# powdr-labs/powdr

Measured on AMD Instinct MI355X. Metric: STARK cells/sec (trace rows x cols) proving guest-keccak [bus interactions (LogUp) inside the proof], higher is better.
Workload: dtype u32 (BabyBear, Montgomery)

## Files before the change

### include/powdr_prover.h

```cpp
#ifndef POWDR_PROVER_H
#define POWDR_PROVER_H

#include <stddef.h>
#include <stdint.h>

#ifdef __cplusplus
extern "C" {
#endif

typedef struct PwProver PwProver;

typedef struct {
    uint32_t num_queries;
    uint32_t pow_bits;
} PwStarkConfig;

PwProver* pw_prover_create(const PwStarkConfig* cfg, uint32_t width, const uint32_t* cons_bytecode,
                           size_t bytecode_len, const uint32_t* cons_spans, size_t n_constraints);
PwProver* pw_prover_create_logup(const PwStarkConfig* cfg, uint32_t width, const uint32_t* cons_bytecode,
                                 size_t bytecode_len, const uint32_t* cons_spans, size_t n_constraints,
                                 const uint32_t* interactions, size_t n_interactions, const uint32_t* inter_spans,
                                 size_t n_inter_spans, const uint32_t* inter_bytecode, size_t inter_bytecode_len);
int pw_prover_trace_root(PwProver* p, const uint32_t* d_trace, uint32_t log_height, uint32_t* root8);
int pw_prover_set_bus_seed(PwProver* p, const uint32_t* seed8);
// ... 225 lines not shown
int pw_prover_stream_log_blocks(const PwProver* p, uint32_t log_height);

int pw_prover_max_constraint_degree(const PwProver* p);

int pw_prover_specialise(PwProver* p);
size_t pw_provers_specialise(PwProver* const* provers, size_t n);
int pw_prover_specialised(const PwProver* p, size_t* n_kernels, size_t* code_bytes, size_t* n_chunks);
size_t pw_jit_generated_source(uint32_t width, const uint32_t* cons_bytecode, size_t bytecode_len, const uint32_t* cons_spans, size_t n_constraints,
                               const uint32_t* interactions, size_t n_interactions, const uint32_t* inter_spans, size_t n_inter_spans,
                               const uint32_t* inter_bytecode, size_t inter_bytecode_len, int which, uint32_t chunk_cost, uint32_t chunks_per_unit,
                               size_t unit, char* buf, size_t cap, char* kernel_name, size_t name_cap, uint32_t* first_chunk, uint32_t* n_chunks,
                               uint32_t* total_chunks);
void pw_jit_cache_stats(uint64_t* units_compiled, uint64_t* units_from_disk);
int pw_jit_compile_check(uint32_t width, const uint32_t* cons_bytecode, size_t bytecode_len, const uint32_t* cons_spans, size_t n_constraints,
                         const uint32_t* interactions, size_t n_interactions, const uint32_t* inter_spans, size_t n_inter_spans,
                         const uint32_t* inter_bytecode, size_t inter_bytecode_len, size_t* n_kernels, size_t* code_bytes, size_t* n_chunks,
                         char* err, size_t err_cap);

uint32_t pw_prover_width(const PwProver* p);

size_t pw_prover_device_bytes(const PwProver* p);


int pw_lde_batch(const uint32_t* d_trace, uint32_t width, uint32_t log_height, uint32_t* d_coeffs, uint32_t* d_lde);

int pw_lde_fused(const uint32_t* d_trace, uint32_t width, uint32_t log_height, uint32_t* d_tmp, uint32_t* d_lde);

int pw_lde_subcoset(const uint32_t* d_coeffs, uint32_t width, uint32_t log_height, uint32_t log_blocks, uint32_t r, uint32_t* d_scale,
                    uint32_t* d_out);

int pw_merkle_commit(const uint32_t* d_matrix, size_t height, uint32_t width, uint32_t* d_digests);

void pw_poseidon2_permute_host(uint32_t* state16);

int pw_set_poseidon2_constants(const uint32_t* ext_rc, const uint32_t* int_rc);
void pw_get_poseidon2_constants(uint32_t* ext_rc, uint32_t* int_rc, uint32_t* diag);

#ifdef __cplusplus
}
#endif
#endif
```

### powdr_amd/csrc/field_selftest.hpp

```cpp
#pragma once
#include "ext.hpp"
#include "poseidon2.hpp"

namespace pw {

PW_HD void selftest_permute_ref(uint32_t* s, const p2::Params& P) {
    auto linear = [&]() {
        uint32_t t[16];
        for (int b = 0; b < 4; ++b) {
            const uint32_t x0 = s[4 * b], x1 = s[4 * b + 1], x2 = s[4 * b + 2], x3 = s[4 * b + 3];
            const uint32_t all = bb::add(bb::add(x0, x1), bb::add(x2, x3));
            t[4 * b] = bb::add(bb::add(all, x0), bb::double_(x1));
            t[4 * b + 1] = bb::add(bb::add(all, x1), bb::double_(x2));
            t[4 * b + 2] = bb::add(bb::add(all, x2), bb::double_(x3));
            t[4 * b + 3] = bb::add(bb::add(all, x3), bb::double_(x0));
        }
        for (int i = 0; i < 4; ++i) {
            const uint32_t col = bb::add(bb::add(t[i], t[4 + i]), bb::add(t[8 + i], t[12 + i]));
            for (int b = 0; b < 4; ++b) s[4 * b + i] = bb::add(t[4 * b + i], col);
        }
    };
    auto sbox = [](uint32_t x) { const uint32_t x2 = bb::mul(x, x), x3 = bb::mul(x2, x), x4 = bb::mul(x2, x2); return bb::mul(x3, x4); };
    linear();
#pragma unroll 1
// ... 168 lines not shown
        }
    }
    if (!params) return 40;
    {
        const uint32_t top = (uint32_t)B::kInputTop - 1;
        const uint32_t mixed[8] = {0u, P - 1, (P - 1) / 2, (P + 1) / 2, P, P + 1, top, 1u};
        const uint32_t n_cases = 2 * (10 + iterations / 64);
#pragma unroll 1
        for (uint32_t c = 0; c < n_cases; ++c) {
            const uint32_t init = c >> 1;
            const int k = (c & 1) ? 3 : 8;
            uint32_t st[16], ref[16], one[16];
            for (int i = 0; i < 16; ++i) {
                st[i] = init == 0 ? 0u : init == 1 ? P - 1 : init == 2 ? (P - 1) / 2 : init == 3 ? (P + 1) / 2 : init == 4 ? mixed[i & 3]
                      : init == 5 ? P : init == 6 ? P + 1 : init == 7 ? top : init == 8 ? mixed[(i * 5 + 4) & 7]
                      : (init & 1) ? rp() : (uint32_t)(rnd() % (uint64_t)B::kInputTop);
                ref[i] = st[i] % P;
            }
#pragma unroll 1
            for (int step = 0; step < 3; ++step) {
                if (step)
                    for (int i = 0; i < k; ++i) st[i] = ref[i] = init < 9 ? mixed[(i + step + init) & 3] : rp();
                for (int i = 0; i < 16; ++i) one[i] = st[i];
                p2::permute<false>(one, *params);
                p2::permute<true>(st, *params);
                selftest_permute_ref(ref, *params);
                for (int i = 0; i < 16; ++i) {
                    if (one[i] != ref[i]) return 38;
                    if (st[i] >= (uint32_t)B::kInputTop || st[i] % P != ref[i]) return 39;
                }
            }
            for (int i = 0; i < 16; ++i)
                if (reduce_2p(st[i]) != ref[i]) return 39;
        }
    }
    for (uint32_t it = 0; it < iterations; ++it) {
        const uint32_t a = rp(), b = rp(), c = rp(), d = rp();
        {
            const int32_t x = (int32_t)((int64_t)(rnd() % (2ull * P + P / 11)) - (int64_t)(P + P / 22));
            uint32_t want = R_MOD_P;
            for (int k = 0; k < 7; ++k) want = mul(want, smodp(x));
            if (smodp(p2::sbox7(x)) != want) return 8;
            const int64_t y = (int64_t)(rnd() % (128ull * P)) - 64ll * P;
            if (smodp(sreduce_wide_loose(y)) != smodp(y)) return 8;
        }
        const uint32_t ab = mul(a, b);
        if (ab >= P || (uint64_t)ab * R_MOD_P % P != (uint64_t)a * b % P) return 10;
        const uint32_t m2 = mul2(a, b, c, d);
        if (m2 != add(ab, mul(c, d))) return 11;
        const uint32_t la = (uint32_t)(rnd() % (2ull * P));
        const uint32_t ml = mul_lazy(la, b);
        if (ml >= 2 * P || ml % P != mul(la % P, b)) return 12;
        if (add_2p(la, (uint32_t)(rnd() % (2ull * P))) >= 2 * P) return 13;
        const uint64_t w = rnd() % (128ull * P);
        if (reduce_wide(w) != w % P) return 14;
        const uint32_t loose = reduce_wide_loose(w);
        if (loose % P != w % P || loose >= (uint64_t)P + P / 32) return 15;
        const uint64_t w16 = rnd() % (16ull * P);
        if (reduce_sum(w16) != w16 % P) return 16;
        if (wide_add(w16, a) != w16 + a || wide_fma(w16, a, 3) != w16 + 3ull * a || wide_mul(a, 4) != 4ull * a) return 17;
        const Ext x{{rp(), rp(), rp(), rp()}}, y{{rp(), rp(), rp(), rp()}}, z{{rp(), rp(), rp(), rp()}};
        if (!ext_eq(ext_mul(ext_mul(x, y), z), ext_mul(x, ext_mul(y, z)))) return 20;
        if (!ext_eq(ext_mul(x, ext_add(y, z)), ext_add(ext_mul(x, y), ext_mul(x, z)))) return 21;
        if ((x.c[0] | x.c[1] | x.c[2] | x.c[3]) && !ext_eq(ext_mul(x, ext_inv(x)), ext_one())) return 22;
        ExtWideAcc acc;
        Ext want = ext_zero();
// ... 41 lines not shown
```

### powdr_amd/csrc/merkle.hip

```cpp
#include "prover_internal.hpp"

#include <algorithm>
#include <cstdlib>
#include <mutex>

namespace pw {

namespace {

constexpr int kBlock = 256;
__constant__ p2::Params c_params;
p2::Params g_host_params;
bool g_params_ready = false;
uint64_t g_params_uploaded = 0;

template <int MINW>
__global__ __launch_bounds__(kBlock, MINW) void leaf_hash_kernel(const uint32_t* __restrict__ m, size_t height,
                                                            uint32_t width, size_t col_stride,
                                                            uint32_t* __restrict__ digests, size_t dstride, size_t doff) {
    const size_t j = (size_t)blockIdx.x * kBlock + threadIdx.x;
    if (j >= height) return;
    uint32_t st[16];
#pragma unroll
    for (int i = 0; i < 16; ++i) st[i] = 0u;
    const uint32_t* col = m + j;
#pragma unroll 1
    for (uint32_t c0 = 0; c0 < width; c0 += 8) {
#pragma unroll
        for (int k = 0; k < 8; ++k)
            if (c0 + k < width) st[k] = col[(size_t)(c0 + k) * col_stride];
        p2::permute<true>(st, c_params);
    }
#pragma unroll
    for (int k = 0; k < 8; ++k) st[k] = bb::reduce_2p(st[k]);
    uint4* out = reinterpret_cast<uint4*>(digests + (j * dstride + doff) * 8);
    out[0] = make_uint4(st[0], st[1], st[2], st[3]);
    out[1] = make_uint4(st[4], st[5], st[6], st[7]);
}

struct LeafLevel {
    const uint32_t* const* cols;
    uint32_t n_cols;
    uint32_t first_block;
    uint64_t height;
    uint32_t* out;
};
struct LeafLevels {
    LeafLevel lv[28];
    int n;
};
template <int MINW>
__global__ __launch_bounds__(kBlock, MINW) void leaf_hash_levels_kernel(const LeafLevels levels) {
    int k = 0;
    while (k + 1 < levels.n && blockIdx.x >= levels.lv[k + 1].first_block) ++k;
    const LeafLevel lv = levels.lv[k];
    const size_t j = (size_t)(blockIdx.x - lv.first_block) * kBlock + threadIdx.x;
    if (j >= lv.height) return;
    uint32_t st[16];
#pragma unroll
    for (int i = 0; i < 16; ++i) st[i] = 0u;
#pragma unroll 1
    for (uint32_t c0 = 0; c0 < lv.n_cols; c0 += 8) {
#pragma unroll
        for (int q = 0; q < 8; ++q)
            if (c0 + q < lv.n_cols) st[q] = lv.cols[c0 + q][j];
        p2::permute<true>(st, c_params);
    }
#pragma unroll
    for (int q = 0; q < 8; ++q) st[q] = bb::reduce_2p(st[q]);
    uint4* out = reinterpret_cast<uint4*>(lv.out + j * 8);
    out[0] = make_uint4(st[0], st[1], st[2], st[3]);
    out[1] = make_uint4(st[4], st[5], st[6], st[7]);
}

struct AbsorbArgs {
    const uint32_t* m;
    size_t col_stride;
    const uint32_t* const* cols;
    uint32_t n_cols, pos0;
    size_t height;
    size_t rstride, roff;
    uint32_t* state;
    uint32_t* digests;
    int first, last;
};
template <int MINW>
__global__ __launch_bounds__(kBlock, MINW) void leaf_absorb_kernel(const AbsorbArgs a) {
    const size_t j = (size_t)blockIdx.x * kBlock + threadIdx.x;
    if (j >= a.height) return;
    const size_t row = j * a.rstride + a.roff;
    uint32_t st[16];
    if (a.first) {
#pragma unroll
        for (int i = 0; i < 16; ++i) st[i] = 0u;
    } else {
        const uint4* in = reinterpret_cast<const uint4*>(a.state + row * 16);
#pragma unroll
        for (int v = 0; v < 4; ++v) { const uint4 x = in[v]; st[4 * v] = x.x; st[4 * v + 1] = x.y; st[4 * v + 2] = x.z; st[4 * v + 3] = x.w; }
    }
    auto cell = [&](uint32_t c) -> uint32_t { return a.cols ? a.cols[c][j] : a.m[(size_t)c * a.col_stride + j]; };
    uint32_t c = 0, pos = a.pos0;
    if (pos) {
#pragma unroll
        for (int k = 0; k < 8; ++k)
            if ((uint32_t)k >= pos && (uint32_t)k - pos < a.n_cols) st[k] = cell((uint32_t)k - pos);
        const uint32_t take = 8u - pos < a.n_cols ? 8u - pos : a.n_cols;
        c = take;
        pos += take;
        if (pos == 8u) { p2::permute<true>(st, c_params); pos = 0; }
    }
#pragma unroll 1
    for (; c < a.n_cols; c += 8) {
#pragma unroll
        for (int k = 0; k < 8; ++k)
            if (c + k < a.n_cols) st[k] = cell(c + k);
        if (c + 8 <= a.n_cols) p2::permute<true>(st, c_params);
        else pos = a.n_cols - c;
    }
    if (a.last) {
        if (pos) p2::permute<true>(st, c_params);
        uint4* out = reinterpret_cast<uint4*>(a.digests + row * 8);
        out[0] = make_uint4(bb::reduce_2p(st[0]), bb::reduce_2p(st[1]), bb::reduce_2p(st[2]), bb::reduce_2p(st[3]));
        out[1] = make_uint4(bb::reduce_2p(st[4]), bb::reduce_2p(st[5]), bb::reduce_2p(st[6]), bb::reduce_2p(st[7]));
    } else {
        uint4* out = reinterpret_cast<uint4*>(a.state + row * 16);
#pragma unroll
        for (int v = 0; v < 4; ++v) out[v] = make_uint4(st[4 * v], st[4 * v + 1], st[4 * v + 2], st[4 * v + 3]);
    }
}

__global__ __launch_bounds__(kBlock) void compress_strided_kernel(const uint32_t* __restrict__ children, size_t n,
                                                                   const uint32_t* __restrict__ inject, uint32_t* __restrict__ parents) {
    const size_t j = (size_t)blockIdx.x * kBlock + threadIdx.x;
    if (j >= n) return;
    const uint4* l = reinterpret_cast<const uint4*>(children + j * 8);
    const uint4* r = reinterpret_cast<const uint4*>(children + (j + n) * 8);
    uint4 a = l[0], b = l[1], c = r[0], d = r[1];
    uint32_t st[16] = {a.x, a.y, a.z, a.w, b.x, b.y, b.z, b.w, c.x, c.y, c.z, c.w, d.x, d.y, d.z, d.w};
    p2::permute(st, c_params);
    if (inject) {
        const uint4* q = reinterpret_cast<const uint4*>(inject + j * 8);
        c = q[0]; d = q[1];
        st[8] = c.x; st[9] = c.y; st[10] = c.z; st[11] = c.w; st[12] = d.x; st[13] = d.y; st[14] = d.z; st[15] = d.w;
        p2::permute(st, c_params);
    }
    uint4* out = reinterpret_cast<uint4*>(parents + j * 8);
    out[0] = make_uint4(st[0], st[1], st[2], st[3]);
    out[1] = make_uint4(st[4], st[5], st[6], st[7]);
}

__global__ __launch_bounds__(kBlock) void ext_pair_leaf_kernel(const bb::Ext* __restrict__ v, size_t half,
                                                                uint32_t* __restrict__ digests) {
    const size_t i = (size_t)blockIdx.x * kBlock + threadIdx.x;
    if (i >= half) return;
    uint32_t st[16];
    const bb::Ext a = v[i], b = v[i + half];
#pragma unroll
    for (int k = 0; k < 4; ++k) { st[k] = a.c[k]; st[4 + k] = b.c[k]; st[8 + k] = 0u; st[12 + k] = 0u; }
// ... 30 lines not shown
    for (int i = 0; i < 8; ++i)
        if ((uint32_t)i == in_len) st[i] = bb::to_monty(w);
    p2::permute(st, c_params);
    const uint32_t sample = st[7];
    if ((bb::from_monty(sample) & ((1u << bits) - 1u)) == 0u) atomicMin(best, w);
}

constexpr size_t kTailNodes = 2048;
__global__ __launch_bounds__(1024) void compress_tail_kernel(uint32_t* __restrict__ digests, size_t n_first, uint32_t* __restrict__ root_out) {
    size_t off = 0;
    for (size_t n = n_first; n > 1; n >>= 1) {
        const size_t parents = n >> 1;
        for (size_t i = threadIdx.x; i < parents; i += 1024) {
            const uint32_t* in = digests + off + i * 16;
            uint32_t st[16];
#pragma unroll
            for (int k = 0; k < 16; ++k) st[k] = in[k];
            p2::permute(st, c_params);
            uint32_t* out = digests + off + n * 8 + i * 8;
#pragma unroll
            for (int k = 0; k < 8; ++k) out[k] = st[k];
        }
        off += n * 8;
        __threadfence_block();
        __syncthreads();
    }
    if (root_out && threadIdx.x < 8) root_out[threadIdx.x] = digests[off + threadIdx.x];
}

int hash_min_waves() {
    const char* e = getenv("POWDR_HASH_WAVES");
    return e ? atoi(e) : 6;
}

struct RootMailbox {
    uint32_t* host = nullptr;
    uint32_t* dev = nullptr;
    int device = -1;
    ~RootMailbox() { if (host) (void)hipHostFree(host); }
};
thread_local RootMailbox g_mailbox;

int build_levels(uint32_t* digests, size_t n_leaves, uint32_t* root_out = nullptr) {
    size_t off = 0;
    size_t n = n_leaves;
    for (; n > kTailNodes; n >>= 1) {
        size_t parents = n >> 1;
        ScopedKernelTimer t("compress_kernel");
        hipLaunchKernelGGL(compress_kernel, dim3(div_up(parents, kBlock)), dim3(kBlock), 0, stream(), digests + off,
                           parents, digests + off + n * 8);
        off += n * 8;
    }
    if (n > 1 || root_out) {
        ScopedKernelTimer t("compress_tail_kernel");
        hipLaunchKernelGGL(compress_tail_kernel, dim3(1), dim3(1024), 0, stream(), digests + off, n, root_out);
    }
    return (int)hipGetLastError();
}

}

static std::mutex g_params_mu;

const p2::Params& poseidon2_params_host() {
    static std::once_flag once;
    std::call_once(once, [] {
// ... 30 lines not shown
    PW_HIP_TRY(hipGetDevice(&device));
    if (device < 64 && (g_params_uploaded >> device) & 1) return 0;
    if (!g_params_ready) { p2::generate_params(g_host_params); g_params_ready = true; }
    const p2::Params& p = g_host_params;
    PW_HIP_TRY(hipDeviceSynchronize());
    PW_HIP_TRY(hipMemcpyToSymbol(HIP_SYMBOL(c_params), &p, sizeof(p2::Params)));
    if (device < 64) g_params_uploaded |= 1ull << device;
    return 0;
}

uint32_t* merkle_root_mailbox(uint32_t** device_ptr) {
    RootMailbox& mb = g_mailbox;
    int device = 0;
    if (hipGetDevice(&device) != hipSuccess) return nullptr;
    if (mb.host && mb.device != device) { (void)hipHostFree(mb.host); mb.host = nullptr; }
    if (!mb.host) {
        void* h = nullptr;
        if (hipHostMalloc(&h, 64, hipHostMallocMapped) != hipSuccess) { (void)hipGetLastError(); return nullptr; }
        void* d = nullptr;
        if (hipHostGetDevicePointer(&d, h, 0) != hipSuccess) { (void)hipGetLastError(); (void)hipHostFree(h); return nullptr; }
        mb.host = (uint32_t*)h; mb.dev = (uint32_t*)d; mb.device = device;
    }
    *device_ptr = mb.dev;
    return mb.host;
}

int merkle_leaf_hash(const uint32_t* m, size_t height, uint32_t width, size_t col_stride, uint32_t* digests, size_t digest_stride,
                     size_t digest_offset) {
    int rc = poseidon2_upload_params();
    if (rc) return rc;
    ScopedKernelTimer t("leaf_hash_kernel");
    if (hash_min_waves() >= 8)
        hipLaunchKernelGGL(leaf_hash_kernel<8>, dim3(div_up(height, kBlock)), dim3(kBlock), 0, stream(), m, height, width, col_stride, digests,
                           digest_stride, digest_offset);
    else
        hipLaunchKernelGGL(leaf_hash_kernel<6>, dim3(div_up(height, kBlock)), dim3(kBlock), 0, stream(), m, height, width, col_stride, digests,
                           digest_stride, digest_offset);
    return (int)hipGetLastError();
}

int merkle_build_levels(uint32_t* digests, size_t n_leaves, uint32_t* root_out) { return build_levels(digests, n_leaves, root_out); }

int merkle_leaf_absorb(const uint32_t* m, size_t col_stride, const uint32_t* const* d_cols, uint32_t n_cols, uint32_t pos0, size_t height, size_t rstride,
                       size_t roff, uint32_t* state, uint32_t* digests, bool first, bool last) {
    int rc = poseidon2_upload_params();
    if (rc) return rc;
    if (!height) return 0;
    const AbsorbArgs a{m, col_stride, d_cols, n_cols, pos0, height, rstride, roff, state, digests, first ? 1 : 0, last ? 1 : 0};
    ScopedKernelTimer t("leaf_hash_kernel");
    if (hash_min_waves() >= 8) hipLaunchKernelGGL(leaf_absorb_kernel<8>, dim3(div_up(height, kBlock)), dim3(kBlock), 0, stream(), a);
    else hipLaunchKernelGGL(leaf_absorb_kernel<6>, dim3(div_up(height, kBlock)), dim3(kBlock), 0, stream(), a);
    return (int)hipGetLastError();
}

int merkle_commit_matrix(const uint32_t* m, size_t height, uint32_t width, size_t col_stride, uint32_t* digests, uint32_t* root_out) {
    const int rc = merkle_leaf_hash(m, height, width, col_stride, digests, 1, 0);
    return rc ? rc : build_levels(digests, height, root_out);
}

int merkle_commit_mixed(const MixedLevelCols* by_log, int L, uint32_t* digests, uint32_t* d_inject) {
    int rc = poseidon2_upload_params();
    if (rc) return rc;
    if (L < 0 || L > 27 || (!by_log[L].n_cols && !by_log[L].external)) return (int)hipErrorInvalidValue;
    const size_t N = (size_t)1 << L;
    LeafLevels levels{};
    LeafLevel* h_levels = levels.lv;
    int n_levels = 0;
    for (int lg = L; lg >= 0; --lg)
        if (by_log[lg].n_cols && !by_log[lg].external)
            h_levels[n_levels++] = LeafLevel{by_log[lg].d_cols, by_log[lg].n_cols, 0u, (uint64_t)1 << lg,
                                             lg == L ? digests : d_inject + ((size_t)1 << lg) * 8};
    std::stable_sort(h_levels, h_levels + n_levels, [](const LeafLevel& a, const LeafLevel& b) { return a.n_cols > b.n_cols; });
    uint32_t blocks = 0;
    for (int k = 0; k < n_levels; ++k) { h_levels[k].first_block = blocks; blocks += div_up((size_t)h_levels[k].height, kBlock); }
    levels.n = n_levels;
    if (n_levels) {
        ScopedKernelTimer t("leaf_hash_kernel");
        if (hash_min_waves() >= 8) hipLaunchKernelGGL(leaf_hash_levels_kernel<8>, dim3(blocks), dim3(kBlock), 0, stream(), levels);
        else hipLaunchKernelGGL(leaf_hash_levels_kernel<6>, dim3(blocks), dim3(kBlock), 0, stream(), levels);
    }
    size_t off = 0;
    for (int lg = L - 1; lg >= 0; --lg) {
        const size_t n = (size_t)1 << lg;
        const uint32_t* inj = (by_log[lg].n_cols || by_log[lg].external) ? d_inject + n * 8 : nullptr;
        ScopedKernelTimer t("compress_kernel");
        hipLaunchKernelGGL(compress_strided_kernel, dim3(div_up(n, kBlock)), dim3(kBlock), 0, stream(), digests + off, n, inj, digests + off + 2 * n * 8);
        off += 2 * n * 8;
    }
    (void)N;
    return (int)hipGetLastError();
}

int merkle_commit_ext_pairs(const bb::Ext* v, size_t half, uint32_t* digests, uint32_t* root_out) {
    int rc = poseidon2_upload_params();
    if (rc) return rc;
    {
        ScopedKernelTimer t("ext_pair_leaf_kernel");
        hipLaunchKernelGGL(ext_pair_leaf_kernel, dim3(div_up(half, kBlock)), dim3(kBlock), 0, stream(), v, half, digests);
    }
    return build_levels(digests, half, root_out);
}

int pow_grind(const uint32_t* d_state16, const uint32_t* d_pending, uint32_t in_len, uint32_t bits, uint32_t* d_best,
              uint32_t* witness_out) {
    int rc = poseidon2_upload_params();
    if (rc) return rc;
    const uint32_t batch = 1u << 20;
    uint32_t best = 0xffffffffu;
// ... 14 lines not shown
```

### powdr_amd/csrc/poseidon2.hpp

```cpp
#pragma once
#include "babybear.hpp"

#ifndef PW_P2_UNROLL
#define PW_P2_UNROLL 1
#endif
#define PW_P2_STR2(x) #x
#define PW_P2_STR(x) PW_P2_STR2(x)
#define PW_P2_ROUND_LOOP _Pragma(PW_P2_STR(unroll PW_P2_UNROLL))
#ifndef PW_P2_UNROLL_PARTIAL
#define PW_P2_UNROLL_PARTIAL 1
#endif
#define PW_P2_PARTIAL_LOOP _Pragma(PW_P2_STR(unroll PW_P2_UNROLL_PARTIAL))

namespace p2 {

namespace bounds {
constexpr int64_t kSmontDomain = 4899916392431616000ll;
constexpr int64_t kSreduceDomain = 257698037888ll;
constexpr int64_t kSreduceE = 134217455ll;
constexpr int64_t kSreduceRound = 2013266050ll;
constexpr int64_t kClosureWide = 191260262495ll;
constexpr int32_t kLayerInTop = 2059960355;
constexpr int32_t kSboxOutTop = 1890224929;
constexpr int64_t kExtWideTop = 87198106825ll;
constexpr int32_t kExtOutTop = 1006632981;
constexpr int32_t kLastInTop = 1419447163;
constexpr int64_t kLastWideLo = 30849986135ll;
constexpr int64_t kLastWideHi = 170476605965ll;
constexpr int32_t kInputTop = 2054886230;
}

struct Params {
    uint32_t ext_rc[8][16];
    uint32_t int_rc[13];
    uint32_t diag[16];
    int64_t ext_fold[8][16];
    int32_t entry_c;
    int32_t part_kappa[2];
    int32_t part_rho[2];
    int32_t part_diag[2][16];
    int64_t int_fold[13];
    int64_t exit_fold[16];
};

inline void default_round_constants(Params& p) {
    uint64_t s = 0x506F736569646F6Eull;
    auto next = [&]() -> uint32_t {
        for (;;) {
            s += 0x9E3779B97F4A7C15ull;
            uint64_t z = s;
            z = (z ^ (z >> 30)) * 0xBF58476D1CE4E5B9ull;
            z = (z ^ (z >> 27)) * 0x94D049BB133111EBull;
            z ^= z >> 31;
            uint32_t v = (uint32_t)(z & 0x7fffffffu);
            if (v < bb::P) return bb::to_monty(v);
        }
    };
    for (int r = 0; r < 8; ++r)
        for (int i = 0; i < 16; ++i) p.ext_rc[r][i] = next();
    for (int r = 0; r < 13; ++r) p.int_rc[r] = next();
}

// ... 76 lines not shown
    constexpr int64_t kBias = 4 * (int64_t)bb::P;
#pragma unroll
    for (int b = 0; b < 4; ++b) {
        const int32_t x0 = s[4 * b], x1 = s[4 * b + 1], x2 = s[4 * b + 2], x3 = s[4 * b + 3];
        const int64_t t01 = bb::swide_add(FOLD ? bb::swide_fma_uniform(fold[4 * b], x0, 1) : BIAS ? bb::swide_fma_uniform(kBias, x0, 1) : bb::swide_mul(x0, 1), x1);
        const int64_t t23 = bb::swide_add(FOLD ? bb::swide_fma_uniform(fold[4 * b + 1], x2, 1) : BIAS ? bb::swide_fma_uniform(kBias, x2, 1) : bb::swide_mul(x2, 1), x3);
        const int64_t t = t01 + t23;
        const int64_t ta = bb::swide_add(t, x1), tb = bb::swide_add(t, x3);
        y[4 * b] = ta + t01;
        y[4 * b + 1] = bb::swide_fma(ta, x2, 2) + (FOLD ? fold[4 * b + 2] : (int64_t)0);
        y[4 * b + 2] = tb + t23;
        y[4 * b + 3] = bb::swide_fma(tb, x0, 2) + (FOLD ? fold[4 * b + 3] : (int64_t)0);
    }
#pragma unroll
    for (int i = 0; i < 4; ++i) {
        const int64_t col = (y[i] + y[4 + i]) + (y[8 + i] + y[12 + i]);
#pragma unroll
        for (int b = 0; b < 4; ++b) s[4 * b + i] = BIAS ? bb::sreduce_wide_loose(y[4 * b + i] + col) : bb::smont(y[4 * b + i] + col);
    }
}

template <bool LAST>
PW_HD void internal_layer(int32_t* s, const int32_t* m, int32_t kappa, int32_t rho, int64_t next_c, const int64_t* exit_c) {
    int64_t wide = bb::smul_uniform(s[0], kappa);
#pragma unroll
    for (int i = 1; i < 16; ++i) wide = bb::swide_add(wide, s[i]);
    const int32_t sum = bb::smont(wide);
    const int64_t sum_r = bb::smul_uniform(sum, rho);
    s[0] = bb::smont(bb::swide_mad_uniform(sum_r + next_c, s[0], m[0]));
#pragma unroll
    for (int i = 1; i < 16; ++i) s[i] = bb::smont(bb::swide_mad_uniform(LAST ? sum_r + exit_c[i] : sum_r, s[i], m[i]));
}

template <bool SPONGE = false>
PW_HD void permute(uint32_t* words, const Params& P) {
    int32_t* s = reinterpret_cast<int32_t*>(words);
    external_layer<true, false>(s, P.ext_fold[0]);
PW_P2_ROUND_LOOP
    for (int r = 0; r < 3; ++r) {
#pragma unroll
        for (int i = 0; i < 16; ++i) s[i] = sbox7(s[i]);
        external_layer<true, false>(s, P.ext_fold[r + 1]);
    }
#pragma unroll
    for (int i = 0; i < 16; ++i) s[i] = sbox7(s[i]);
    external_layer<false, false>(s, nullptr);
    s[0] += P.entry_c;
    s[0] = sbox7(s[0]);
    internal_layer<false>(s, P.part_diag[0], P.part_kappa[0], P.part_rho[0], P.int_fold[0], nullptr);
PW_P2_PARTIAL_LOOP
    for (int r = 1; r < 12; ++r) {
        s[0] = sbox7(s[0]);
        internal_layer<false>(s, P.part_diag[1], P.part_kappa[1], P.part_rho[1], P.int_fold[r], nullptr);
    }
    s[0] = sbox7(s[0]);
    internal_layer<true>(s, P.part_diag[1], P.part_kappa[1], P.part_rho[1], P.int_fold[12], P.exit_fold);
PW_P2_ROUND_LOOP
    for (int r = 4; r < 7; ++r) {
#pragma unroll
        for (int i = 0; i < 16; ++i) s[i] = sbox7(s[i]);
        external_layer<true, false>(s, P.ext_fold[r + 1]);
    }
#pragma unroll
    for (int i = 0; i < 16; ++i) s[i] = sbox7(s[i]);
    external_layer<false, true>(s, nullptr);
    if (!SPONGE) {
#pragma unroll
        for (int i = 0; i < 16; ++i) words[i] = bb::reduce_2p(words[i]);
    }
}

}
```

### powdr_amd/csrc/prover.hip

```cpp
#include "prover_state.hpp"
#include "prover_stages.hpp"
#include "xbc_compile.hpp"

#include <atomic>
#include <cstdlib>
#include <cstring>
#include <algorithm>
#include <initializer_list>
#include <vector>

namespace pw {

namespace {

__global__ void gather_records_kernel(const uint32_t* __restrict__ arena, const uint64_t* __restrict__ offsets,
                                      uint32_t words_per_record, uint32_t n, uint32_t* __restrict__ out) {
    const uint32_t i = blockIdx.x * blockDim.x + threadIdx.x;
    if (i >= n * words_per_record) return;
    const uint32_t r = i / words_per_record, w = i - r * words_per_record;
    out[i] = arena[offsets[r] + w];
}

}

// ... 883 lines not shown
extern "C" int pw_lde_subcoset(const uint32_t* d_coeffs, uint32_t width, uint32_t log_h, uint32_t log_blocks, uint32_t r, uint32_t* d_scale,
                               uint32_t* d_out) {
    (void)hipGetLastError();
    if (!d_coeffs || !d_scale || !d_out || !width || log_blocks < 1 || log_blocks > log_h || log_h > 26 || (r >> log_blocks)) return -1;
    if ((uintptr_t)d_coeffs & 15) return (int)hipErrorInvalidValue;
    const size_t H = (size_t)1 << log_h, m = (2 * H) >> log_blocks;
    TRY(subcoset_lde(d_coeffs, d_out, H, m, width, (int)log_h, (int)log_blocks, r, d_scale));
    return (int)hipGetLastError();
}

extern "C" int pw_merkle_commit(const uint32_t* d_matrix, size_t height, uint32_t width, uint32_t* d_digests) {
    (void)hipGetLastError();
    if (!height || (height & (height - 1))) return -1;
    return merkle_commit_matrix(d_matrix, height, width, height, d_digests);
}

extern "C" int pw_set_poseidon2_constants(const uint32_t* ext_rc, const uint32_t* int_rc) {
    return poseidon2_set_constants(ext_rc, int_rc);
}

extern "C" void pw_get_poseidon2_constants(uint32_t* ext_rc, uint32_t* int_rc, uint32_t* diag) {
    const p2::Params& p = poseidon2_params_host();
    if (ext_rc) for (int r = 0; r < 8; ++r) for (int i = 0; i < 16; ++i) ext_rc[16 * r + i] = bb::from_monty(p.ext_rc[r][i]);
    if (int_rc) for (int r = 0; r < 13; ++r) int_rc[r] = bb::from_monty(p.int_rc[r]);
    if (diag) for (int i = 0; i < 16; ++i) diag[i] = bb::from_monty(p.diag[i]);
}

extern "C" void pw_poseidon2_permute_host(uint32_t* s) {
    uint32_t m[16];
    for (int i = 0; i < 16; ++i) m[i] = bb::to_monty(s[i] % bb::P);
    p2::permute(m, poseidon2_params_host());
    for (int i = 0; i < 16; ++i) s[i] = bb::from_monty(m[i]);
}
```

### rust/powdr-hip/src/ffi.rs

```rust
#![allow(non_camel_case_types, clippy::too_many_arguments)]

use core::ffi::{c_char, c_int, c_uint, c_void};

pub type PowdrFp = u32;

#[repr(C)]
#[derive(Clone, Copy, Debug)]
pub struct OriginalAir {
    pub width: i32,
    pub height: i32,
    pub buffer: *const PowdrFp,
    pub row_block_size: i32,
}
#[repr(C)]
#[derive(Clone, Copy, Debug)]
pub struct Subst {
    pub air_index: i32,
    pub col: i32,
    pub row: i32,
    pub apc_col: i32,
}
#[repr(C)]
#[derive(Clone, Copy)]
pub struct ExprSpan {
// ... 449 lines not shown
                                   n_links: usize, where_: *mut usize) -> c_int;
    pub fn pw_prove_airs(airs: *const PwSegmentAir, n_airs: usize, shared_bus_seed: c_int, n_workers: c_uint,
                         proofs: *mut *const u32, n_words: *mut usize, bus_seed8: *mut u32) -> c_int;
    pub fn pw_verify_airs(cfg: *const PwStarkConfig, airs: *const PwAirDescription, n_airs: usize,
                          proofs: *const *const u32, n_words: *const usize, shared_bus_seed: c_int,
                          check_balance: c_int, total_sum4: *mut u32) -> c_int;
    pub fn pw_commitment_digest(roots8: *const u32, n: usize, digest8: *mut u32);
    pub fn pw_prover_reserve(p: *mut PwProver, log_height: u32) -> c_int;
    pub fn pw_prover_stream_log_blocks(p: *const PwProver, log_height: u32) -> c_int;
    pub fn pw_prover_max_constraint_degree(p: *const PwProver) -> c_int;
    pub fn pw_prover_width(p: *const PwProver) -> u32;
    pub fn pw_prover_device_bytes(p: *const PwProver) -> usize;
    pub fn pw_lde_batch(d_trace: *const u32, width: u32, log_height: u32, d_coeffs: *mut u32, d_lde: *mut u32) -> c_int;
    pub fn pw_lde_fused(d_trace: *const u32, width: u32, log_height: u32, d_tmp: *mut u32, d_lde: *mut u32) -> c_int;
    pub fn pw_lde_subcoset(d_coeffs: *const u32, width: u32, log_height: u32, log_blocks: u32, r: u32, d_scale: *mut u32, d_out: *mut u32) -> c_int;
    pub fn pw_merkle_commit(d_matrix: *const u32, height: usize, width: u32, d_digests: *mut u32) -> c_int;
    pub fn pw_prover_specialise(p: *mut PwProver) -> c_int;
    pub fn pw_prover_specialised(p: *const PwProver, n_kernels: *mut usize, code_bytes: *mut usize, n_chunks: *mut usize) -> c_int;
    pub fn pw_prove_segments_multi(devices: *const c_int, n_workers: usize, segment_cells: *const u64, n_segments: usize,
                                   prove: PwSegmentProveFn, user: *mut c_void, commitments: *mut u32, worker_of_segment: *mut u32) -> c_int;
    pub fn pw_multi_last_merge() -> c_int;
    pub fn pw_assign_units(cells: *const u64, n_units: usize, n_workers: usize, worker_of_unit: *mut u32) -> usize;
    pub fn pw_jit_generated_source(width: u32, cons_bytecode: *const u32, bytecode_len: usize, cons_spans: *const u32, n_constraints: usize,
                                   interactions: *const u32, n_interactions: usize, inter_spans: *const u32, n_inter_spans: usize,
                                   inter_bytecode: *const u32, inter_bytecode_len: usize, which: c_int, chunk_cost: u32, chunks_per_unit: u32,
                                   unit: usize, buf: *mut c_char, cap: usize, kernel_name: *mut c_char, name_cap: usize, first_chunk: *mut u32,
                                   n_chunks: *mut u32, total_chunks: *mut u32) -> usize;
    pub fn pw_jit_cache_stats(units_compiled: *mut u64, units_from_disk: *mut u64);
    pub fn pw_jit_compile_check(width: u32, cons_bytecode: *const u32, bytecode_len: usize, cons_spans: *const u32, n_constraints: usize,
                                interactions: *const u32, n_interactions: usize, inter_spans: *const u32, n_inter_spans: usize,
                                inter_bytecode: *const u32, inter_bytecode_len: usize, n_kernels: *mut usize, code_bytes: *mut usize,
                                n_chunks: *mut usize, err: *mut c_char, err_cap: usize) -> c_int;
    pub fn pw_poseidon2_permute_host(state16: *mut u32);
    pub fn pw_set_poseidon2_constants(ext_rc: *const u32, int_rc: *const u32) -> c_int;
    pub fn pw_get_poseidon2_constants(ext_rc: *mut u32, int_rc: *mut u32, diag: *mut u32);
}

extern "C" {
    pub fn hipMalloc(ptr: *mut *mut c_void, bytes: usize) -> c_int;
    pub fn hipFree(ptr: *mut c_void) -> c_int;
    pub fn hipMemcpy(dst: *mut c_void, src: *const c_void, bytes: usize, kind: c_int) -> c_int;
    pub fn hipMemset(dst: *mut c_void, value: c_int, bytes: usize) -> c_int;
    pub fn hipDeviceSynchronize() -> c_int;
    pub fn hipSetDevice(device: c_int) -> c_int;
}
pub const HIP_MEMCPY_HOST_TO_DEVICE: c_int = 1;
pub const HIP_MEMCPY_DEVICE_TO_HOST: c_int = 2;
```

Measured before the change: 7.164 billion.

## Merge Poseidon2 sponge boundary layers across absorbed blocks in leaf hashing

Restructures the leaf-hash sponge so that between consecutive absorbed blocks the final external linear layer of one permutation and the entry external layer of the next are fused into an open-form combination with wide signed accumulators. This avoids a full reduce-then-relinearise step per block. The three leaf hash kernels now share one absorb_run helper that uses address-space-typed loads, block-base column pointers plus a lane offset, and scheduling fences. A POWDR_HASH_CLOSED env knob keeps the old closed form, and a host reference digest and selftests are added. The risk is extra register pressure from the 64-bit intermediates in a kernel that is already occupancy-sensitive.

```diff
diff --git a/include/powdr_prover.h b/include/powdr_prover.h
--- a/include/powdr_prover.h
+++ b/include/powdr_prover.h
@@ -281,6 +281,7 @@
 int pw_merkle_commit(const uint32_t* d_matrix, size_t height, uint32_t width, uint32_t* d_digests);
 
 void pw_poseidon2_permute_host(uint32_t* state16);
+void pw_poseidon2_row_digest_host(const uint32_t* row, uint32_t width, int closed, uint32_t* digest8);
 
 int pw_set_poseidon2_constants(const uint32_t* ext_rc, const uint32_t* int_rc);
 void pw_get_poseidon2_constants(uint32_t* ext_rc, uint32_t* int_rc, uint32_t* diag);
diff --git a/powdr_amd/csrc/field_selftest.hpp b/powdr_amd/csrc/field_selftest.hpp
--- a/powdr_amd/csrc/field_selftest.hpp
+++ b/powdr_amd/csrc/field_selftest.hpp
@@ -224,6 +224,115 @@
             }
             for (int i = 0; i < 16; ++i)
                 if (reduce_2p(st[i]) != ref[i]) return 39;
+        }
+    }
+    {
+        auto layer_ref = [&](const uint64_t* x, const int64_t* fold, uint64_t* want) {
+            for (int q = 0; q < 4; ++q) {
+                const uint64_t x0 = x[4 * q], x1 = x[4 * q + 1], x2 = x[4 * q + 2], x3 = x[4 * q + 3];
+                const uint64_t a = fold ? smodp(fold[4 * q]) : 0, b = fold ? smodp(fold[4 * q + 1]) : 0;
+                const uint64_t d1 = fold ? smodp(fold[4 * q + 2]) : 0, d3 = fold ? smodp(fold[4 * q + 3]) : 0;
+                want[4 * q] = (2 * x0 + 3 * x1 + x2 + x3 + 2 * a + b) % P;
+                want[4 * q + 1] = (x0 + 2 * x1 + 3 * x2 + x3 + a + b + d1) % P;
+                want[4 * q + 2] = (x0 + x1 + 2 * x2 + 3 * x3 + a + 2 * b) % P;
+                want[4 * q + 3] = (3 * x0 + x1 + x2 + 2 * x3 + a + b + d3) % P;
+            }
+            for (int i = 0; i < 4; ++i) {
+                const uint64_t col = want[i] + want[4 + i] + want[8 + i] + want[12 + i];
+                for (int q = 0; q < 4; ++q) want[4 * q + i] = (want[4 * q + i] + col) % P;
+            }
+        };
+#pragma unroll 1
+        for (int sp = 0; sp < 5; ++sp) {
+            int32_t t[16];
+            uint64_t x[16], want[16];
+            for (int i = 0; i < 16; ++i) {
+                const bool neg = sp == 1 || (sp == 2 && (i & 1)) || (sp == 3 && ((i >> 2) & 1)) || (sp == 4 && (rnd() & 1));
+                const int32_t mag = sp == 4 ? (int32_t)(rnd() % (uint64_t)B::kLastInTop) : B::kLastInTop - 1;
+                t[i] = neg ? -mag : mag;
+                x[i] = smodp(t[i]);
+            }
+            layer_ref(x, nullptr, want);
+            int64_t o[8];
+            p2::last_layer_open(t, o);
+            for (int i = 0; i < 8; ++i) {
+                if (smodp(o[i]) != want[8 + i] || o[i] >= B::kOpenTop || o[i] <= -B::kOpenTop) return 41;
+                if (sp < 2 && o[i] != (sp ? -1 : 1) * (B::kOpenTop - 35)) return 41;
+            }
+        }
+#pragma unroll 1
+        for (int pat = 0; pat < 5 * 5 * 4; ++pat) {
+            const int sp = pat % 5, fr = (pat / 5) % 5, fp = pat / 25;
+            int64_t o[8], fold[16];
+            int32_t s[16];
+            uint64_t x[16], want[16];
+            for (int i = 0; i < 16; ++i) {
+                const bool neg = sp == 1 || (sp == 2 && (i & 1)) || (sp == 3 && ((i >> 2) & 1)) || (sp == 4 && (rnd() & 1));
+                if (i < 8) {
+                    s[i] = fr == 0 ? 0 : fr == 1 ? 1 : fr == 2 ? (int32_t)(P - 1) : fr == 3 ? B::kLayerInTop - 1 : (int32_t)rp();
+                    x[i] = smodp(s[i]);
+                } else {
+                    const int64_t mag = sp == 4 ? (int64_t)(rnd() % (uint64_t)B::kOpenTop) : B::kOpenTop - 1;
+                    o[i - 8] = neg ? -mag : mag;
+                    x[i] = smodp(o[i - 8]);
+                    s[i] = 0x7fffffff;
+                }
+                fold[i] = fp == 0 ? HALF : fp == 1 ? -HALF : fp == 2 ? (neg ? -HALF : HALF) : centred(rp());
+            }
+            layer_ref(x, fold, want);
+            p2::entry_layer_open(s, o, fold);
+            for (int i = 0; i < 16; ++i) {
+                if ((uint64_t)smodp(s[i]) * R_MOD_P % P != want[i]) return 42;
+                if (s[i] >= B::kEntryOutTop || s[i] <= -B::kEntryOutTop) return 43;
+            }
+        }
+        const uint32_t edge_words[4] = {0u, 1u, P - 1, (P - 1) / 2};
+#pragma unroll 1
+        for (int c = 0; c < 3 * 5 * 2; ++c) {
+            const int n = (c % 3) == 0 ? 2 : (c % 3) == 1 ? 3 : 5, kind = (c / 3) % 5, init = c / 15;
+            uint32_t blocks[5][8];
+            for (int b = 0; b < 5; ++b)
+                for (int k = 0; k < 8; ++k) blocks[b][k] = kind < 3 ? edge_words[kind] : kind == 3 ? edge_words[(b + 3 * k) & 3] : rp();
+            uint32_t first[16];
+            for (int i = 0; i < 16; ++i) first[i] = i < 8 ? blocks[0][i] : init ? (uint32_t)B::kInputTop - 1 : 0u;
+#pragma unroll 1
+            for (int form = 0; form < 4; ++form) {
+                const int short_k = form == 3 ? 3 : 8;
+                uint32_t one[16], st[16];
+                for (int i = 0; i < 16; ++i) { one[i] = first[i] % P; st[i] = first[i]; }
+                if (form == 0) {
+                    int32_t* s = reinterpret_cast<int32_t*>(st);
+                    p2::external_layer<true, false>(s, params->ext_fold[0]);
+#pragma unroll 1
+                    for (int b = 0; b < n; ++b) {
+                        p2::rounds(s, *params);
+                        p2::permute<false>(one, *params);
+                        if (b + 1 == n) break;
+                        int64_t o[8];
+                        p2::last_layer_open(s, o);
+                        for (int i = 0; i < 8; ++i)
+                            if (smodp(o[i]) != one[8 + i] || o[i] >= B::kOpenTop || o[i] <= -B::kOpenTop) return 44;
+                        for (int k = 0; k < 8; ++k) { s[k] = (int32_t)blocks[b + 1][k]; one[k] = blocks[b + 1][k]; }
+                        p2::entry_layer_open(s, o, params->ext_fold[0]);
+                        for (int i = 0; i < 16; ++i)
+                            if (s[i] >= B::kEntryOutTop || s[i] <= -B::kEntryOutTop) return 44;
+                    }
+                    p2::external_layer<false, true>(s, nullptr);
+                } else {
+#pragma unroll 1
+                    for (int b = 0; b < n; ++b) {
+                        if (b)
+                            for (int k = 0; k < (b + 1 == n ? short_k : 8); ++k) one[k] = blocks[b][k];
+                        p2::permute<false>(one, *params);
+                    }
+                    const uint32_t n_merged = form == 2 ? 0u : form == 3 ? (uint32_t)n - 2u : (uint32_t)n - 1u;
+                    p2::absorb_blocks(st, (uint32_t)n, n_merged, *params,
+                                      [&](uint32_t b, uint32_t* fresh) { for (int k = 0; k < 8; ++k) fresh[k] = blocks[b][k]; },
+                                      [&](uint32_t b, uint32_t* words) { for (int k = 0; k < (b + 1 == (uint32_t)n ? short_k : 8); ++k) words[k] = blocks[b][k]; });
+                }
+                for (int i = 0; i < 16; ++i)
+                    if (st[i] >= (uint32_t)B::kInputTop || reduce_2p(st[i]) != one[i]) return 45 + (form > 1 ? 2 : form);
+            }
         }
     }
     for (uint32_t it = 0; it < iterations; ++it) {
diff --git a/powdr_amd/csrc/merkle.hip b/powdr_amd/csrc/merkle.hip
--- a/powdr_amd/csrc/merkle.hip
+++ b/powdr_amd/csrc/merkle.hip
@@ -1,6 +1,7 @@
 #include "prover_internal.hpp"
 
 #include <algorithm>
+#include <cstddef>
 #include <cstdlib>
 #include <mutex>
 
@@ -14,28 +15,54 @@
 bool g_params_ready = false;
 uint64_t g_params_uploaded = 0;
 
+typedef const __attribute__((address_space(1))) char* GlobalBytes;
+typedef const __attribute__((address_space(4))) uint64_t* ConstantWords;
+__device__ __forceinline__ uint32_t cell_ld(const uint32_t* base, uint32_t off4) {
+    return *reinterpret_cast<const __attribute__((address_space(1))) uint32_t*>((GlobalBytes)(uintptr_t)base + off4);
+}
+__device__ __forceinline__ uint32_t lane_offset() {
+    uint32_t off4 = 4u * threadIdx.x;
+    asm volatile("" : "+v"(off4));
+    return off4;
+}
+__device__ __forceinline__ const uint32_t* column_ptr(const uint32_t* const* cols, uint32_t c) {
+    return reinterpret_cast<const uint32_t*>((uintptr_t)((ConstantWords)(uintptr_t)cols)[c]);
+}
+
+template <class ColBase>
+struct LaneCells {
+    ColBase col_base;
+    __device__ __forceinline__ uint32_t block() const { return lane_offset(); }
+    __device__ __forceinline__ uint32_t at(uint32_t c, uint32_t off4) const { return cell_ld(col_base(c), off4); }
+};
+template <class ColBase>
+__device__ __forceinline__ void absorb_run(uint32_t* st, uint32_t pos0, uint32_t n_cols, bool last, bool closed, ColBase col_base) {
+    p2::absorb_run(st, pos0, n_cols, last, closed, c_params, LaneCells<ColBase>{col_base});
+}
+
+__device__ __forceinline__ uint32_t thread_again() {
+    uint32_t t = threadIdx.x;
+    asm volatile("" : "+v"(t));
+    return t;
+}
+
+__device__ __forceinline__ void store_digest(uint32_t* out8, const uint32_t* st) {
+    uint4* out = reinterpret_cast<uint4*>(out8);
+    out[0] = make_uint4(bb::reduce_2p(st[0]), bb::reduce_2p(st[1]), bb::reduce_2p(st[2]), bb::reduce_2p(st[3]));
+    out[1] = make_uint4(bb::reduce_2p(st[4]), bb::reduce_2p(st[5]), bb::reduce_2p(st[6]), bb::reduce_2p(st[7]));
+}
+
 template <int MINW>
 __global__ __launch_bounds__(kBlock, MINW) void leaf_hash_kernel(const uint32_t* __restrict__ m, size_t height,
                                                             uint32_t width, size_t col_stride,
-                                                            uint32_t* __restrict__ digests, size_t dstride, size_t doff) {
-    const size_t j = (size_t)blockIdx.x * kBlock + threadIdx.x;
+                                                            uint32_t* __restrict__ digests, size_t dstride, size_t doff, int closed) {
+    const size_t j0 = (size_t)blockIdx.x * kBlock, j = j0 + threadIdx.x;
     if (j >= height) return;
     uint32_t st[16];
 #pragma unroll
     for (int i = 0; i < 16; ++i) st[i] = 0u;
-    const uint32_t* col = m + j;
-#pragma unroll 1
-    for (uint32_t c0 = 0; c0 < width; c0 += 8) {
-#pragma unroll
-        for (int k = 0; k < 8; ++k)
-            if (c0 + k < width) st[k] = col[(size_t)(c0 + k) * col_stride];
-        p2::permute<true>(st, c_params);
-    }
-#pragma unroll
-    for (int k = 0; k < 8; ++k) st[k] = bb::reduce_2p(st[k]);
-    uint4* out = reinterpret_cast<uint4*>(digests + (j * dstride + doff) * 8);
-    out[0] = make_uint4(st[0], st[1], st[2], st[3]);
-    out[1] = make_uint4(st[4], st[5], st[6], st[7]);
+    absorb_run(st, 0u, width, true, closed != 0, [&](uint32_t c) { return m + j0 + (size_t)c * col_stride; });
+    store_digest(digests + ((j0 + thread_again()) * dstride + doff) * 8, st);
 }
 
 struct LeafLevel {
@@ -48,29 +75,21 @@
 struct LeafLevels {
     LeafLevel lv[28];
     int n;
+    int closed;
 };
 template <int MINW>
 __global__ __launch_bounds__(kBlock, MINW) void leaf_hash_levels_kernel(const LeafLevels levels) {
     int k = 0;
     while (k + 1 < levels.n && blockIdx.x >= levels.lv[k + 1].first_block) ++k;
     const LeafLevel lv = levels.lv[k];
-    const size_t j = (size_t)(blockIdx.x - lv.first_block) * kBlock + threadIdx.x;
+    const size_t j0 = (size_t)(blockIdx.x - lv.first_block) * kBlock, j = j0 + threadIdx.x;
     if (j >= lv.height) return;
     uint32_t st[16];
 #pragma unroll
     for (int i = 0; i < 16; ++i) st[i] = 0u;
-#pragma unroll 1
-    for (uint32_t c0 = 0; c0 < lv.n_cols; c0 += 8) {
-#pragma unroll
-        for (int q = 0; q < 8; ++q)
-            if (c0 + q < lv.n_cols) st[q] = lv.cols[c0 + q][j];
-        p2::permute<true>(st, c_params);
-    }
-#pragma unroll
-    for (int q = 0; q < 8; ++q) st[q] = bb::reduce_2p(st[q]);
-    uint4* out = reinterpret_cast<uint4*>(lv.out + j * 8);
-    out[0] = make_uint4(st[0], st[1], st[2], st[3]);
-    out[1] = make_uint4(st[4], st[5], st[6], st[7]);
+    const uint32_t* const* cols = lv.cols;
+    absorb_run(st, 0u, lv.n_cols, true, levels.closed != 0, [&](uint32_t c) { return column_ptr(cols, c) + j0; });
+    store_digest(lv.out + (j0 + thread_again()) * 8, st);
 }
 
 struct AbsorbArgs {
@@ -83,10 +102,11 @@
     uint32_t* state;
     uint32_t* digests;
     int first, last;
+    int closed;
 };
 template <int MINW>
 __global__ __launch_bounds__(kBlock, MINW) void leaf_absorb_kernel(const AbsorbArgs a) {
-    const size_t j = (size_t)blockIdx.x * kBlock + threadIdx.x;
+    const size_t j0 = (size_t)blockIdx.x * kBlock, j = j0 + threadIdx.x;
     if (j >= a.height) return;
     const size_t row = j * a.rstride + a.roff;
     uint32_t st[16];
@@ -98,32 +118,17 @@
 #pragma unroll
         for (int v = 0; v < 4; ++v) { const uint4 x = in[v]; st[4 * v] = x.x; st[4 * v + 1] = x.y; st[4 * v + 2] = x.z; st[4 * v + 3] = x.w; }
     }
-    auto cell = [&](uint32_t c) -> uint32_t { return a.cols ? a.cols[c][j] : a.m[(size_t)c * a.col_stride + j]; };
-    uint32_t c = 0, pos = a.pos0;
-    if (pos) {
-#pragma unroll
-        for (int k = 0; k < 8; ++k)
-            if ((uint32_t)k >= pos && (uint32_t)k - pos < a.n_cols) st[k] = cell((uint32_t)k - pos);
-        const uint32_t take = 8u - pos < a.n_cols ? 8u - pos : a.n_cols;
-        c = take;
-        pos += take;
-        if (pos == 8u) { p2::permute<true>(st, c_params); pos = 0; }
-    }
-#pragma unroll 1
-    for (; c < a.n_cols; c += 8) {
-#pragma unroll
-        for (int k = 0; k < 8; ++k)
-            if (c + k < a.n_cols) st[k] = cell(c + k);
-        if (c + 8 <= a.n_cols) p2::permute<true>(st, c_params);
-        else pos = a.n_cols - c;
-    }
+    static_assert(offsetof(AbsorbArgs, m) == 0, "the kernel's argument block must begin with the matrix pointer");
+    const uint32_t* const* table = a.cols ? a.cols : (const uint32_t* const*)(uintptr_t)__builtin_amdgcn_kernarg_segment_ptr();
+    const uint32_t table_mask = a.cols ? ~0u : 0u;
+    const size_t stride = a.cols ? 0 : a.col_stride;
+    absorb_run(st, a.pos0, a.n_cols, a.last != 0, a.closed != 0,
+               [&](uint32_t c) { return column_ptr(table, c & table_mask) + (size_t)c * stride + j0; });
+    const size_t row_out = (j0 + thread_again()) * a.rstride + a.roff;
     if (a.last) {
-        if (pos) p2::permute<true>(st, c_params);
-        uint4* out = reinterpret_cast<uint4*>(a.digests + row * 8);
-        out[0] = make_uint4(bb::reduce_2p(st[0]), bb::reduce_2p(st[1]), bb::reduce_2p(st[2]), bb::reduce_2p(st[3]));
-        out[1] = make_uint4(bb::reduce_2p(st[4]), bb::reduce_2p(st[5]), bb::reduce_2p(st[6]), bb::reduce_2p(st[7]));
+        store_digest(a.digests + row_out * 8, st);
     } else {
-        uint4* out = reinterpret_cast<uint4*>(a.state + row * 16);
+        uint4* out = reinterpret_cast<uint4*>(a.state + row_out * 16);
 #pragma unroll
         for (int v = 0; v < 4; ++v) out[v] = make_uint4(st[4 * v], st[4 * v + 1], st[4 * v + 2], st[4 * v + 3]);
     }
@@ -220,6 +225,10 @@
     const char* e = getenv("POWDR_HASH_WAVES");
     return e ? atoi(e) : 6;
 }
+int hash_closed() {
+    const char* e = getenv("POWDR_HASH_CLOSED");
+    return e && atoi(e) ? 1 : 0;
+}
 
 struct RootMailbox {
     uint32_t* host = nullptr;
@@ -316,10 +325,10 @@
     ScopedKernelTimer t("leaf_hash_kernel");
     if (hash_min_waves() >= 8)
         hipLaunchKernelGGL(leaf_hash_kernel<8>, dim3(div_up(height, kBlock)), dim3(kBlock), 0, stream(), m, height, width, col_stride, digests,
-                           digest_stride, digest_offset);
+                           digest_stride, digest_offset, hash_closed());
     else
         hipLaunchKernelGGL(leaf_hash_kernel<6>, dim3(div_up(height, kBlock)), dim3(kBlock), 0, stream(), m, height, width, col_stride, digests,
-                           digest_stride, digest_offset);
+                           digest_stride, digest_offset, hash_closed());
     return (int)hipGetLastError();
 }
 
@@ -330,7 +339,7 @@
     int rc = poseidon2_upload_params();
     if (rc) return rc;
     if (!height) return 0;
-    const AbsorbArgs a{m, col_stride, d_cols, n_cols, pos0, height, rstride, roff, state, digests, first ? 1 : 0, last ? 1 : 0};
+    const AbsorbArgs a{m, col_stride, d_cols, n_cols, pos0, height, rstride, roff, state, digests, first ? 1 : 0, last ? 1 : 0, hash_closed()};
     ScopedKernelTimer t("leaf_hash_kernel");
     if (hash_min_waves() >= 8) hipLaunchKernelGGL(leaf_absorb_kernel<8>, dim3(div_up(height, kBlock)), dim3(kBlock), 0, stream(), a);
     else hipLaunchKernelGGL(leaf_absorb_kernel<6>, dim3(div_up(height, kBlock)), dim3(kBlock), 0, stream(), a);
@@ -358,6 +367,7 @@
     uint32_t blocks = 0;
     for (int k = 0; k < n_levels; ++k) { h_levels[k].first_block = blocks; blocks += div_up((size_t)h_levels[k].height, kBlock); }
     levels.n = n_levels;
+    levels.closed = hash_closed();
     if (n_levels) {
         ScopedKernelTimer t("leaf_hash_kernel");
         if (hash_min_waves() >= 8) hipLaunchKernelGGL(leaf_hash_levels_kernel<8>, dim3(blocks), dim3(kBlock), 0, stream(), levels);
diff --git a/powdr_amd/csrc/poseidon2.hpp b/powdr_amd/csrc/poseidon2.hpp
--- a/powdr_amd/csrc/poseidon2.hpp
+++ b/powdr_amd/csrc/poseidon2.hpp
@@ -28,6 +28,9 @@
 constexpr int64_t kLastWideLo = 30849986135ll;
 constexpr int64_t kLastWideHi = 170476605965ll;
 constexpr int32_t kInputTop = 2054886230;
+constexpr int64_t kOpenTop = 49680650705ll;
+constexpr int64_t kEntryWideTop = 1087232604175ll;
+constexpr int32_t kEntryOutTop = 1006633214;
 }
 
 struct Params {
@@ -170,10 +173,7 @@
     for (int i = 1; i < 16; ++i) s[i] = bb::smont(bb::swide_mad_uniform(LAST ? sum_r + exit_c[i] : sum_r, s[i], m[i]));
 }
 
-template <bool SPONGE = false>
-PW_HD void permute(uint32_t* words, const Params& P) {
-    int32_t* s = reinterpret_cast<int32_t*>(words);
-    external_layer<true, false>(s, P.ext_fold[0]);
+PW_HD void rounds(int32_t* s, const Params& P) {
 PW_P2_ROUND_LOOP
     for (int r = 0; r < 3; ++r) {
 #pragma unroll
@@ -193,14 +193,21 @@
     }
     s[0] = sbox7(s[0]);
     internal_layer<true>(s, P.part_diag[1], P.part_kappa[1], P.part_rho[1], P.int_fold[12], P.exit_fold);
+#pragma unroll
+    for (int i = 0; i < 16; ++i) s[i] = sbox7(s[i]);
 PW_P2_ROUND_LOOP
-    for (int r = 4; r < 7; ++r) {
+    for (int r = 5; r < 8; ++r) {
+        external_layer<true, false>(s, P.ext_fold[r]);
 #pragma unroll
         for (int i = 0; i < 16; ++i) s[i] = sbox7(s[i]);
-        external_layer<true, false>(s, P.ext_fold[r + 1]);
-    }
-#pragma unroll
-    for (int i = 0; i < 16; ++i) s[i] = sbox7(s[i]);
+    }
+}
+
+template <bool SPONGE = false>
+PW_HD void permute(uint32_t* words, const Params& P) {
+    int32_t* s = reinterpret_cast<int32_t*>(words);
+    external_layer<true, false>(s, P.ext_fold[0]);
+    rounds(s, P);
     external_layer<false, true>(s, nullptr);
     if (!SPONGE) {
 #pragma unroll
@@ -208,4 +215,130 @@
     }
 }
 
-}
+PW_HD void last_layer_open(const int32_t* t, int64_t* o) {
+    int64_t y[16];
+#pragma unroll
+    for (int b = 0; b < 4; ++b) {
+        const int32_t x0 = t[4 * b], x1 = t[4 * b + 1], x2 = t[4 * b + 2], x3 = t[4 * b + 3];
+        const int64_t t01 = bb::swide_add(bb::swide_mul(x0, 1), x1);
+        const int64_t t23 = bb::swide_add(bb::swide_mul(x2, 1), x3);
+        const int64_t s = t01 + t23;
+        const int64_t ta = bb::swide_add(s, x1), tb = bb::swide_add(s, x3);
+        y[4 * b] = ta + t01;
+        y[4 * b + 1] = bb::swide_fma(ta, x2, 2);
+        y[4 * b + 2] = tb + t23;
+        y[4 * b + 3] = bb::swide_fma(tb, x0, 2);
+    }
+#pragma unroll
+    for (int i = 0; i < 4; ++i) {
+        const int64_t col = (y[i] + y[4 + i]) + (y[8 + i] + y[12 + i]);
+        o[i] = y[8 + i] + col;
+        o[4 + i] = y[12 + i] + col;
+    }
+}
+
+PW_HD void entry_layer_open(int32_t* s, const int64_t* o, const int64_t* fold) {
+    int64_t y[16];
+#pragma unroll
+    for (int b = 0; b < 2; ++b) {
+        const int32_t x0 = s[4 * b], x1 = s[4 * b + 1], x2 = s[4 * b + 2], x3 = s[4 * b + 3];
+        const int64_t t01 = bb::swide_add(bb::swide_fma_uniform(fold[4 * b], x0, 1), x1);
+        const int64_t t23 = bb::swide_add(bb::swide_fma_uniform(fold[4 * b + 1], x2, 1), x3);
+        const int64_t t = t01 + t23;
+        const int64_t ta = bb::swide_add(t, x1), tb = bb::swide_add(t, x3);
+        y[4 * b] = ta + t01;
+        y[4 * b + 1] = bb::swide_fma(ta, x2, 2) + fold[4 * b + 2];
+        y[4 * b + 2] = tb + t23;
+        y[4 * b + 3] = bb::swide_fma(tb, x0, 2) + fold[4 * b + 3];
+    }
+#pragma unroll
+    for (int b = 2; b < 4; ++b) {
+        const int64_t x0 = o[4 * b - 8], x1 = o[4 * b - 7], x2 = o[4 * b - 6], x3 = o[4 * b - 5];
+        const int64_t t01 = (x0 + fold[4 * b]) + x1;
+        const int64_t t23 = (x2 + fold[4 * b + 1]) + x3;
+        const int64_t t = t01 + t23;
+        const int64_t ta = t + x1, tb = t + x3;
+        y[4 * b] = ta + t01;
+        y[4 * b + 1] = (ta + 2 * x2) + fold[4 * b + 2];
+        y[4 * b + 2] = tb + t23;
+        y[4 * b + 3] = (tb + 2 * x0) + fold[4 * b + 3];
+    }
+#pragma unroll
+    for (int i = 0; i < 4; ++i) {
+        const int64_t col = (y[i] + y[4 + i]) + (y[8 + i] + y[12 + i]);
+#pragma unroll
+        for (int b = 0; b < 4; ++b) s[4 * b + i] = bb::smont(y[4 * b + i] + col);
+    }
+}
+
+PW_HD const Params& table_view(const Params& P) {
+#if defined(__HIP_DEVICE_COMPILE__)
+    uint32_t zero = 0;
+    asm volatile("" : "+s"(zero));
+    return *reinterpret_cast<const Params*>(reinterpret_cast<const char*>(&P) + zero);
+#else
+    return P;
+#endif
+}
+
+PW_HD void phase_fence() {
+#if defined(__HIP_DEVICE_COMPILE__)
+    __builtin_amdgcn_sched_barrier(0);
+#endif
+}
+
+template <class LoadFull, class LoadRate>
+PW_HD void absorb_blocks(uint32_t* words, uint32_t n_perm, uint32_t n_merged, const Params& P, LoadFull&& load_full, LoadRate&& load_rate) {
+    int32_t* s = reinterpret_cast<int32_t*>(words);
+    external_layer<true, false>(s, P.ext_fold[0]);
+#pragma unroll 1
+    for (uint32_t b = 1;; ++b) {
+        rounds(s, table_view(P));
+        if (b >= n_perm) break;
+        const Params& Q = table_view(P);
+        if (b <= n_merged) {
+            uint32_t fresh[8];
+            load_full(b, fresh);
+            int64_t o[8];
+            phase_fence();
+            last_layer_open(s, o);
+            phase_fence();
+#pragma unroll
+            for (int k = 0; k < 8; ++k) s[k] = (int32_t)fresh[k];
+            entry_layer_open(s, o, Q.ext_fold[0]);
+            phase_fence();
+        } else {
+            external_layer<false, true>(s, nullptr);
+            load_rate(b, words);
+            external_layer<true, false>(s, Q.ext_fold[0]);
+        }
+    }
+    external_layer<false, true>(s, nullptr);
+}
+
+template <class Cells>
+PW_HD void absorb_run(uint32_t* st, uint32_t pos0, uint32_t n_cols, bool last, bool closed, const Params& P, const Cells& cells) {
+    const uint32_t total = pos0 + n_cols, n_full = total >> 3, tail = total & 7u;
+    const uint32_t n_perm = n_full + (last && tail ? 1u : 0u);
+    auto load_rate = [&](uint32_t b, uint32_t* words) {
+        const auto t = cells.block();
+#pragma unroll
+        for (uint32_t k = 0; k < 8; ++k) {
+            const uint32_t c = 8u * b + k - pos0;
+            if (c < n_cols) words[k] = cells.at(c, t);
+        }
+    };
+    auto load_full = [&](uint32_t b, uint32_t* fresh) {
+        const uint32_t c0 = 8u * b - pos0;
+        const auto t = cells.block();
+#pragma unroll
+        for (uint32_t k = 0; k < 8; ++k) fresh[k] = cells.at(c0 + k, t);
+    };
+    if (n_perm) {
+        load_rate(0u, st);
+        absorb_blocks(st, n_perm, closed || !n_full ? 0u : n_full - 1u, P, load_full, load_rate);
+    }
+    if (tail && !last) load_rate(n_full, st);
+}
+
+}
diff --git a/powdr_amd/csrc/prover.hip b/powdr_amd/csrc/prover.hip
--- a/powdr_amd/csrc/prover.hip
+++ b/powdr_amd/csrc/prover.hip
@@ -939,3 +939,14 @@
     p2::permute(m, poseidon2_params_host());
     for (int i = 0; i < 16; ++i) s[i] = bb::from_monty(m[i]);
 }
+
+extern "C" void pw_poseidon2_row_digest_host(const uint32_t* row, uint32_t width, int closed, uint32_t* digest8) {
+    struct RowCells {
+        const uint32_t* words;
+        int block() const { return 0; }
+        uint32_t at(uint32_t c, int) const { return bb::to_monty(words[c] % bb::P); }
+    };
+    uint32_t st[16] = {0};
+    p2::absorb_run(st, 0u, width, true, closed != 0, poseidon2_params_host(), RowCells{row});
+    for (int i = 0; i < 8; ++i) digest8[i] = bb::from_monty(bb::reduce_2p(st[i]));
+}
diff --git a/rust/powdr-hip/src/ffi.rs b/rust/powdr-hip/src/ffi.rs
--- a/rust/powdr-hip/src/ffi.rs
+++ b/rust/powdr-hip/src/ffi.rs
@@ -505,6 +505,7 @@
                                 inter_bytecode: *const u32, inter_bytecode_len: usize, n_kernels: *mut usize, code_bytes: *mut usize,
                                 n_chunks: *mut usize, err: *mut c_char, err_cap: usize) -> c_int;
     pub fn pw_poseidon2_permute_host(state16: *mut u32);
+    pub fn pw_poseidon2_row_digest_host(row: *const u32, width: u32, closed: c_int, digest8: *mut u32);
     pub fn pw_set_poseidon2_constants(ext_rc: *const u32, int_rc: *const u32) -> c_int;
     pub fn pw_get_poseidon2_constants(ext_rc: *mut u32, int_rc: *mut u32, diag: *mut u32);
 }
```

After: 7.214 billion, median of 6. Within noise of the previous version (+0.7%).
